# emdgroup/tnmf

Hardware: AMD Instinct MI355X
Metric: MU-iterations/sec (higher is better)
Workload: dtype f32

## Files before the change

### tnmf_amd/csrc/fft.h

```cpp
#pragma once
#include "common.h"

struct FftArgs {
    const void *src0, *src1, *src2;
    void *dst0, *dst1;
    long ps_src, ps_dst;
    int planes, rows, cols;
    int ld_src, ld_dst;
    int KX, KXP;
    int yoff, xoff;
    int N, M, C, Hy;
    int n0, ngroups, nper;
    int mgroups, mper;
    int clamp0;
    double reg;
};

enum FftOp {
    kFftRowsFwd = 0,
    kFftRowsInv,
    kFftRowsInv2,
    kFftRowsMu,
    kFftColsFwd,
    kFftColsInv,
    kFftContractR,
    kFftGradH,
    kFftGradW,
};

typedef int (*fft_run_fn)(int op, int dtype, const FftArgs *a, hipStream_t s);
#define TNMF_FFT_DECL(L) int fft_run_##L(int op, int dtype, const FftArgs *a, hipStream_t s)
TNMF_FFT_DECL(32);
TNMF_FFT_DECL(48);
TNMF_FFT_DECL(64);
TNMF_FFT_DECL(96);
TNMF_FFT_DECL(144);
TNMF_FFT_DECL(192);
TNMF_FFT_DECL(270);
TNMF_FFT_DECL(288);
TNMF_FFT_DECL(384);
TNMF_FFT_DECL(540);
TNMF_FFT_DECL(576);
#undef TNMF_FFT_DECL

bool mixed_has_reconstruct(const Geo &g, int dtype);
bool mixed_has_grad_W(const Geo &g, int dtype);
int mixed_reconstruct(const Geo &g, const void *Tsp, const void *WT, void *OT, int KX, int KXP, hipStream_t s);
int mixed_grad_W(const Geo &g, const void *Tsp, const void *VT, const void *RT, void *Gn, void *Gp, int KX, int KXP,
                 int ngroups, int nper, hipStream_t s);

int spectral_contract_R(const Geo &g, int dtype, const void *SH, const void *SW, void *SR, int Ly, int KX, int KXP,
                        hipStream_t s);
int spectral_grad_W(const Geo &g, int dtype, const void *SH, const void *SV, const void *SR, void *Gn, void *Gp, int Ly,
                    int KX, int KXP, int ngroups, int nper, hipStream_t s);

bool fft_has(const Geo &g, int dtype);
void fft_invalidate(tnmf_hip_ctx *ctx);
void fft_invalidate_H(tnmf_hip_ctx *ctx, const Geo &g, int dtype, const void *H);
void fft_bind(tnmf_hip_ctx *ctx, const Geo &g, int dtype, const void *H, const void *V);
void fft_unbind(tnmf_hip_ctx *ctx);
void fft_invalidate_W(tnmf_hip_ctx *ctx);
void fft_release(tnmf_hip_ctx *ctx);
int fft_reserve(tnmf_hip_ctx *ctx, const Geo &g, int dtype, bool with_window);

int fft_reconstruct(tnmf_hip_ctx *ctx, const Geo &g, int dtype, const void *W, const void *H, void *R, bool nonneg,
                    hipStream_t s);
int fft_grad_H(tnmf_hip_ctx *ctx, const Geo &g, int dtype, const void *V, const void *R, const void *W, void *neg,
               void *pos, hipStream_t s);
int fft_update_H(tnmf_hip_ctx *ctx, const Geo &g, int dtype, const void *V, const void *R, const void *W, void *H,
                 double reg, hipStream_t s);
int fft_grad_W(tnmf_hip_ctx *ctx, const Geo &g, int dtype, const void *V, const void *R, const void *H, void *neg,
               void *pos, bool nonneg, hipStream_t s);
```

### tnmf_amd/csrc/fft.hip

```cpp
#include <algorithm>
#include <cstdlib>

#include "fft.h"
#include "fft_engine.h"

namespace {

const int kLensY[] = {32, 48, 64, 96, 144, 192, 270, 288, 384, 576};
const int kLensX[] = {32, 48, 64, 96, 144, 192, 270, 288, 384, 540, 576};
constexpr int kMixMaxGroups = 128;

int pick_len(int h, int dtype, bool along_x, bool tall = false) {
    if (along_x || tall) {
        for (int L : kLensX)
            if (L >= h && (dtype == 0 || L <= 288)) return L;
        return 0;
    }
    for (int L : kLensY)
        if (L >= h && (dtype == 0 || L <= 288)) return L;
    return 0;
}

bool tall_columns(const tnmf_hip_ctx *ctx) { return ctx->path != TNMF_PATH_FFT; }

// ... 372 lines not shown
    a.planes = planes;
    a.rows = rows;
    a.cols = cols;
    a.ld_src = cols;
    a.ps_src = (long)rows * cols;
    a.ps_dst = (long)rows * l.KXP;
    return l.rowf(kFftRowsFwd, dtype, &a, s);
}

int columns_of(const Geo &g, const Lay &l, int dtype, const void *Tsrc, int planes, int rows, void *S, hipStream_t s) {
    FftArgs b = base_args(g, l);
    b.src0 = Tsrc;
    b.dst0 = S;
    b.planes = planes;
    b.rows = rows;
    return l.colf(kFftColsFwd, dtype, &b, s);
}

int spectra_V(tnmf_hip_ctx *ctx, const Geo &g, const Call &c, int dtype, const void *V, bool full, hipStream_t s) {
    FftState &f = ctx->fft;
    const Lay &l = c.l;
    const bool track = c.sl.v_cached && f.cache_enabled;
    const bool hit = track && all_ok(f.V_ok, c.sl.n0, g.N);
    ++(hit ? f.v_hits : f.v_runs);
    if (!track && c.sl.cached) {
        set_ok(f.V_ok, c.sl.n0, g.N, 0);
        set_ok(f.SV_ok, c.sl.n0, g.N, 0);
    }
    if (!hit) {
        if (track) {
            set_ok(f.V_ok, c.sl.n0, g.N, 0);
            set_ok(f.SV_ok, c.sl.n0, g.N, 0);
        }
        CHECK(forward_rows(g, l, dtype, V, g.N * g.C, g.Dy, g.Dx, c.VT, s));
        if (track) set_ok(f.V_ok, c.sl.n0, g.N, 1);
    }
    if (full && !(hit && all_ok(f.SV_ok, c.sl.n0, g.N))) {
        CHECK(columns_of(g, l, dtype, c.VT, g.N * g.C, g.Dy, c.SV, s));
        if (track) set_ok(f.SV_ok, c.sl.n0, g.N, 1);
    }
    return TNMF_OK;
}

int rows_of_H(tnmf_hip_ctx *ctx, const Geo &g, const Call &c, int dtype, const void *H, hipStream_t s) {
    FftState &f = ctx->fft;
    const bool track = c.sl.cached && f.cache_enabled;
    if (track && all_ok(f.T_ok, c.sl.n0, g.N)) {
        ++f.h_hits;
        return TNMF_OK;
    }
    ++f.h_runs;
    if (track) {
        set_ok(f.T_ok, c.sl.n0, g.N, 0);
        set_ok(f.SH_ok, c.sl.n0, g.N, 0);
    }
    FftArgs a = base_args(g, c.l);
    a.src0 = H;
    a.dst0 = c.T;
    a.planes = g.N * g.M;
    a.rows = g.Hy;
    a.cols = g.Hx;
    a.ld_src = g.Hs;
    a.ps_src = (long)g.Hy * g.Hs;
    a.ps_dst = (long)g.Hy * c.l.KXP;
    CHECK(c.l.rowf(kFftRowsFwd, dtype, &a, s));
    if (track) set_ok(f.T_ok, c.sl.n0, g.N, 1);
    return TNMF_OK;
}

int spectra_of_H(tnmf_hip_ctx *ctx, const Geo &g, const Call &c, int dtype, const void *H, hipStream_t s) {
    FftState &f = ctx->fft;
    CHECK(rows_of_H(ctx, g, c, dtype, H, s));
    const bool track = c.sl.cached && f.cache_enabled;
    if (track && all_ok(f.SH_ok, c.sl.n0, g.N)) return TNMF_OK;
    CHECK(columns_of(g, c.l, dtype, c.T, g.N * g.M, g.Hy, c.SH, s));
    if (track) set_ok(f.SH_ok, c.sl.n0, g.N, 1);
    return TNMF_OK;
}

}

bool fft_has(const Geo &g, int dtype) {
    if (g.Dy == 1 && g.Ay == 1) {
        return pick_len(g.Hx, dtype, true) != 0 && mixed_has_reconstruct(g, dtype) && mixed_has_grad_W(g, dtype);
    }
    return pick_len(g.Hy, dtype, false) != 0 && pick_len(g.Hx, dtype, true) != 0;
}

void fft_bind(tnmf_hip_ctx *ctx, const Geo &g, int dtype, const void *H, const void *V) {
    bind(ctx->fft, g, dtype, H, V, true);
}

void fft_unbind(tnmf_hip_ctx *ctx) {
    FftState &f = ctx->fft;
    f.bound = f.explicit_bind = false;
    f.H_base = f.V_base = nullptr;
    f.T_ok.clear();
    f.SH_ok.clear();
    f.V_ok.clear();
    f.SV_ok.clear();
}

void fft_invalidate_H(tnmf_hip_ctx *ctx, const Geo &g, int dtype, const void *H) {
    FftState &f = ctx->fft;
    const Slot sl = locate(f, g, dtype, H, nullptr);
    if (sl.cached) {
        set_ok(f.T_ok, sl.n0, g.N, 0);
        set_ok(f.SH_ok, sl.n0, g.N, 0);
    } else {
        std::fill(f.T_ok.begin(), f.T_ok.end(), 0);
        std::fill(f.SH_ok.begin(), f.SH_ok.end(), 0);
    }
}

void fft_invalidate(tnmf_hip_ctx *ctx) { clear_flags(ctx->fft); }

void fft_invalidate_W(tnmf_hip_ctx *ctx) { ctx->fft.W_ok = false; }

int fft_reserve(tnmf_hip_ctx *ctx, const Geo &g, int dtype, bool with_window) {
    Lay l;
    ctx->fft.failed_bytes = 0;
    const FftState &f = ctx->fft;
    const bool in_binding = f.bound && f.dtype == dtype && same_shape(f.geo, g) && f.geo.N >= g.N;
    if (!fft_has(g, dtype) || !make_layout(ctx, in_binding ? f.geo : g, g, dtype, &l)) return TNMF_E_UNSUPPORTED;
    return ensure_ws(ctx, with_window ? l.total : l.total_no_window);
}

void fft_release(tnmf_hip_ctx *ctx) {
    if (ctx->fft.ws) (void)hipFree(ctx->fft.ws);
    ctx->fft.ws = nullptr;
    ctx->fft.ws_bytes = 0;
    ctx->fft.failed_bytes = 0;
    clear_flags(ctx->fft);
}

int fft_reconstruct(tnmf_hip_ctx *ctx, const Geo &g, int dtype, const void *W, const void *H, void *R, bool nonneg,
                    hipStream_t s) {
    Call c;
    CHECK(prepare(ctx, g, dtype, H, nullptr, &c));
    const Lay &l = c.l;
    CHECK(rows_of_H(ctx, g, c, dtype, H, s));
    FftState &f = ctx->fft;
    const bool w_hit = f.cache_enabled && f.W_ok && f.W_owner == W && f.W_dtype == dtype && same_shape(f.W_geo, g) &&
                       (c.sl.cached || f.W_geo.N == g.N);
    auto w_mark = [&]() {
        f.W_ok = f.cache_enabled;
        f.W_owner = W;
        f.W_geo = g;
        f.W_dtype = dtype;
    };
    if (use_mixed(g, dtype, false)) {
        if (!w_hit) {
            f.W_ok = false;
            CHECK(scaled_W(ctx, g, l, dtype, W, 1.0 / l.Lx, s));
            CHECK(forward_rows(g, l, dtype, at(ctx, l.Wt), g.M * g.C, g.Ay, g.Ax, at(ctx, l.TWr), s));
            w_mark();
        }
        CHECK(mixed_reconstruct(g, c.T, at(ctx, l.TWr), c.Ts, l.KX, l.KXP, s));
    } else {
        if (!w_hit) {
            f.W_ok = false;
            CHECK(spectra_W(ctx, g, l, dtype, W, true, false, s));
            w_mark();
        }
        if (use_resident(l)) {
            CHECK(spectra_of_H(ctx, g, c, dtype, H, s));
            CHECK(spectral_contract_R(g, dtype, c.SH, at(ctx, l.SW), c.SR, l.Ly, l.KX, l.KXP, s));
        } else {
            FftArgs a = base_args(g, l);
            a.src0 = c.T;
            a.src1 = at(ctx, l.SW);
            a.dst0 = c.SR;
            CHECK(l.colf(kFftContractR, dtype, &a, s));
        }
        FftArgs b = base_args(g, l);
        b.src0 = c.SR;
        b.dst0 = c.Ts;
        b.planes = g.N * g.C;
        b.rows = g.Dy;
        b.yoff = g.Ay - 1;
        CHECK(l.colf(kFftColsInv, dtype, &b, s));
    }
    FftArgs d = base_args(g, l);
    d.src0 = c.Ts;
    d.dst0 = R;
    d.planes = g.N * g.C;
    d.rows = g.Dy;
    d.cols = g.Dx;
    d.xoff = g.Ax - 1;
    d.ld_dst = g.Dx;
    d.ps_dst = (long)g.Dy * g.Dx;
    d.clamp0 = nonneg ? 1 : 0;
    return l.rowf(kFftRowsInv, dtype, &d, s);
}

namespace {

int grad_H_spectra(tnmf_hip_ctx *ctx, const Geo &g, const Call &c, int dtype, const void *V, const void *R,
                   const void *W, hipStream_t s) {
    CHECK(spectra_W(ctx, g, c.l, dtype, W, false, true, s));
    CHECK(spectra_V(ctx, g, c, dtype, V, true, s));
    return forward_planes(g, c.l, dtype, R, g.N * g.C, g.Dy, g.Dx, c.Ts, c.SR, s);
}

int grad_H_window(tnmf_hip_ctx *ctx, const Geo &g, const Call &c, int dtype, int n0, int cnt, hipStream_t s) {
    const Lay &l = c.l;
    FftArgs a = base_args(g, l);
    a.src0 = c.SV;
    a.src1 = c.SR;
    a.src2 = at(ctx, l.SWf);
    a.dst0 = at(ctx, l.Tn);
    a.dst1 = at(ctx, l.Tp);
    a.n0 = n0;
    a.planes = cnt;
    a.mgroups = l.mgroups;
    a.mper = l.mper;
    return l.colf(kFftGradH, dtype, &a, s);
}

}

int fft_grad_H(tnmf_hip_ctx *ctx, const Geo &g, int dtype, const void *V, const void *R, const void *W, void *neg,
               void *pos, hipStream_t s) {
    if (g.Dy == 1 && g.Ay == 1) return TNMF_E_UNSUPPORTED;
    Call c;
    CHECK(prepare(ctx, g, dtype, nullptr, V, &c, true));
    const Lay &l = c.l;
    CHECK(grad_H_spectra(ctx, g, c, dtype, V, R, W, s));
    const size_t esz = l.csz / 2, hplane = (size_t)g.M * g.Hy * g.Hx;
    for (int n0 = 0; n0 < g.N; n0 += l.chunk) {
        const int cnt = g.N - n0 < l.chunk ? g.N - n0 : l.chunk;
        CHECK(grad_H_window(ctx, g, c, dtype, n0, cnt, s));
        FftArgs a = base_args(g, l);
        a.src0 = at(ctx, l.Tn);
        a.src1 = at(ctx, l.Tp);
        a.dst0 = static_cast<char *>(neg) + (size_t)n0 * hplane * esz;
        a.dst1 = static_cast<char *>(pos) + (size_t)n0 * hplane * esz;
        a.planes = cnt * g.M;
        a.rows = g.Hy;
        a.cols = g.Hx;
        a.xoff = 0;
        a.ld_dst = g.Hx;
        a.ps_dst = (long)g.Hy * g.Hx;
        CHECK(l.rowf(kFftRowsInv2, dtype, &a, s));
    }
    return TNMF_OK;
}

int fft_update_H(tnmf_hip_ctx *ctx, const Geo &g, int dtype, const void *V, const void *R, const void *W, void *H,
                 double reg, hipStream_t s) {
    if (g.Dy == 1 && g.Ay == 1) return TNMF_E_UNSUPPORTED;
    Call c;
    CHECK(prepare(ctx, g, dtype, H, V, &c, true));
    const Lay &l = c.l;
    FftState &f = ctx->fft;
    const bool track = c.sl.cached && f.cache_enabled;
    CHECK(grad_H_spectra(ctx, g, c, dtype, V, R, W, s));
    if (track) {
        set_ok(f.T_ok, c.sl.n0, g.N, 0);
        set_ok(f.SH_ok, c.sl.n0, g.N, 0);
    }
    const size_t esz = l.csz / 2, hplane = (size_t)g.M * g.Hy * g.Hs;
    for (int n0 = 0; n0 < g.N; n0 += l.chunk) {
        const int cnt = g.N - n0 < l.chunk ? g.N - n0 : l.chunk;
        CHECK(grad_H_window(ctx, g, c, dtype, n0, cnt, s));
        FftArgs a = base_args(g, l);
        a.src0 = at(ctx, l.Tn);
        a.src1 = at(ctx, l.Tp);
        a.dst0 = static_cast<char *>(H) + (size_t)n0 * hplane * esz;
        a.dst1 = c.T + (size_t)n0 * l.sT;
        a.planes = cnt * g.M;
        a.rows = g.Hy;
        a.cols = g.Hx;
        a.ld_dst = g.Hs;
        a.ps_src = (long)g.Hy * g.Hs;
        a.ps_dst = (long)g.Hy * l.KXP;
        a.reg = reg;
        CHECK(l.rowf(kFftRowsMu, dtype, &a, s));
    }
    if (track) set_ok(f.T_ok, c.sl.n0, g.N, 1);
    return TNMF_OK;
}

int mix_groups(const tnmf_hip_ctx *ctx, const Geo &g, const Lay &l) {
    const long slots = 2L * 4 * (ctx->num_cu > 0 ? ctx->num_cu : 256);
    const long per_group_block = (long)(g.C == 1 && g.Ay <= 12 ? cdiv(g.M, 2) : g.M) * cdiv(l.KX, 16);
    int best = 32;
    double best_cost = 1e30;
    for (int cand = 32; cand <= kMixMaxGroups; cand *= 2) {
        int ng = g.N < cand ? g.N : cand;
        const int nper = cdiv(g.N, ng);
        ng = cdiv(g.N, nper);
        const double rounds = (double)(per_group_block * cdiv(ng, 4)) / (double)slots;
        const double whole = rounds <= 1.0 ? 1.0 : (double)(long)(rounds + 0.999999);
        const double cost = whole / rounds + 0.03 * (cand / 32);
        if (cost < best_cost - 1e-9) {
            best_cost = cost;
            best = cand;
        }
    }
    return best;
}

int fft_grad_W(tnmf_hip_ctx *ctx, const Geo &g, int dtype, const void *V, const void *R, const void *H, void *neg,
               void *pos, bool nonneg, hipStream_t s) {
    Call c;
    CHECK(prepare(ctx, g, dtype, H, V, &c));
    const Lay &l = c.l;
    CHECK(rows_of_H(ctx, g, c, dtype, H, s));
    const bool mixed = use_mixed(g, dtype, true);
    CHECK(spectra_V(ctx, g, c, dtype, V, !mixed, s));
    const int planes = 2 * g.M * g.C;
    if (mixed) {
        CHECK(forward_rows(g, l, dtype, R, g.N * g.C, g.Dy, g.Dx, c.RT, s));
        int ng_want = mix_groups(ctx, g, l);
        if (const char *e = tnmf_diag_env("TNMF_MIX_GROUPS")) ng_want = atoi(e);
        ng_want = ng_want < 1 ? 1 : (ng_want > kMixMaxGroups ? kMixMaxGroups : ng_want);
        int ng = g.N < ng_want ? g.N : ng_want;
        const int nper = cdiv(g.N, ng);
        ng = cdiv(g.N, nper);
        const int ngpad = (int)align_up((size_t)ng, 4);
        CHECK(mixed_grad_W(g, c.T, c.VT, c.RT, at(ctx, l.Gn), at(ctx, l.Gp), l.KX, l.KXP, ngpad, nper, s));
        const long count = (long)g.M * g.C * g.Ay * l.KXP;
        char *out = at(ctx, l.TW);
        hipLaunchKernelGGL(k_fft_sum_groups<float>, dim3((unsigned)((count + 63) / 64), 2), dim3(64), 0, s,
                           (const cplx<float> *)at(ctx, l.Gn), (const cplx<float> *)at(ctx, l.Gp), (cplx<float> *)out,
                           (cplx<float> *)(out + (size_t)count * l.csz), count, ngpad, 1.0 / l.Lx);
        TNMF_LAUNCH_CHECK();
    } else {
        CHECK(forward_planes(g, l, dtype, R, g.N * g.C, g.Dy, g.Dx, c.Ts, c.SR, s));
        int ngroups = l.ngroups;
        if (use_resident(l)) {
            CHECK(spectra_of_H(ctx, g, c, dtype, H, s));
            const long blocks = (long)cdiv(g.M, 4) * (((long)l.Ly * l.KXP + 255) / 256) * cdiv(g.C, 4);
            int ng = (int)((8L * ctx->num_cu + blocks - 1) / blocks);
            ng = ng < 1 ? 1 : (ng > l.ngroups ? l.ngroups : ng);
            const int nper = cdiv(g.N, ng);
            ngroups = cdiv(g.N, nper);
            CHECK(spectral_grad_W(g, dtype, c.SH, c.SV, c.SR, at(ctx, l.Gn), at(ctx, l.Gp), l.Ly, l.KX, l.KXP, ngroups,
                                  nper, s));
        } else {
            FftArgs a = base_args(g, l);
            a.src0 = c.T;
            a.src1 = c.SV;
            a.src2 = c.SR;
            a.dst0 = at(ctx, l.Gn);
            a.dst1 = at(ctx, l.Gp);
            a.ngroups = l.ngroups;
            a.nper = l.nper;
            CHECK(l.colf(kFftGradW, dtype, &a, s));
        }
        const long count = (long)g.M * g.C * l.Ly * l.KXP;
        const size_t sbytes = (size_t)count * l.csz;
        const double scale = 1.0 / ((double)l.Ly * l.Lx);
        {
            char *out = at(ctx, l.Gs);
            const dim3 grid((unsigned)((count + 63) / 64), 2);
            if (dtype == 0)
                hipLaunchKernelGGL(k_fft_sum_groups<float>, grid, dim3(64), 0, s, (const cplx<float> *)at(ctx, l.Gn),
                                   (const cplx<float> *)at(ctx, l.Gp), (cplx<float> *)out, (cplx<float> *)(out + sbytes),
                                   count, ngroups, scale);
            else
                hipLaunchKernelGGL(k_fft_sum_groups<double>, grid, dim3(64), 0, s, (const cplx<double> *)at(ctx, l.Gn),
                                   (const cplx<double> *)at(ctx, l.Gp), (cplx<double> *)out,
                                   (cplx<double> *)(out + sbytes), count, ngroups, scale);
            TNMF_LAUNCH_CHECK();
        }
        FftArgs b = base_args(g, l);
        b.src0 = at(ctx, l.Gs);
        b.dst0 = at(ctx, l.TW);
        b.planes = planes;
        b.rows = g.Ay;
        b.yoff = 0;
        CHECK(l.colf(kFftColsInv, dtype, &b, s));
    }
    FftArgs d = base_args(g, l);
    d.src0 = at(ctx, l.TW);
    d.dst0 = at(ctx, l.Wo);
    d.planes = planes;
    d.rows = g.Ay;
    d.cols = g.Ax;
    d.xoff = 0;
    d.ld_dst = g.Ax;
    d.ps_dst = (long)g.Ay * g.Ax;
    CHECK(l.rowf(kFftRowsInv, dtype, &d, s));
    const int per = g.M * g.C * g.Ay * g.Ax;
    const char *wo = at(ctx, l.Wo);
    if (dtype == 0) {
        hipLaunchKernelGGL(k_fft_flip_out<float>, dim3(cdiv(per, 256)), dim3(256), 0, s, (const float *)wo,
                           (float *)neg, g.M * g.C, g.Ay, g.Ax, nonneg ? 1 : 0);
        hipLaunchKernelGGL(k_fft_flip_out<float>, dim3(cdiv(per, 256)), dim3(256), 0, s, (const float *)wo + per,
                           (float *)pos, g.M * g.C, g.Ay, g.Ax, nonneg ? 1 : 0);
    } else {
        hipLaunchKernelGGL(k_fft_flip_out<double>, dim3(cdiv(per, 256)), dim3(256), 0, s, (const double *)wo,
                           (double *)neg, g.M * g.C, g.Ay, g.Ax, nonneg ? 1 : 0);
        hipLaunchKernelGGL(k_fft_flip_out<double>, dim3(cdiv(per, 256)), dim3(256), 0, s, (const double *)wo + per,
                           (double *)pos, g.M * g.C, g.Ay, g.Ax, nonneg ? 1 : 0);
    }
    TNMF_LAUNCH_CHECK();
    return TNMF_OK;
}
```

### tnmf_amd/csrc/fft_mixed.hip

```cpp
#include "fft.h"

namespace {

typedef float f2v __attribute__((ext_vector_type(2)));
template <typename T>
struct cplx_of;
template <>
struct cplx_of<float> {
    using type = f2v;
};
template <typename T>
using cplx = typename cplx_of<T>::type;

__device__ __forceinline__ void cfma(f2v &acc, f2v a, f2v b) {
    asm("v_pk_fma_f32 %0, %1, %2, %0 op_sel:[0,0,0] op_sel_hi:[0,1,1]" : "+v"(acc) : "v"(a), "v"(b));
    asm("v_pk_fma_f32 %0, %1, %2, %0 op_sel:[1,1,0] op_sel_hi:[1,0,1] neg_lo:[0,1,0]" : "+v"(acc) : "v"(a), "v"(b));
}
__device__ __forceinline__ void cfmac(f2v &acc, f2v a, f2v b) {
    asm("v_pk_fma_f32 %0, %1, %2, %0 op_sel:[0,0,0] op_sel_hi:[0,1,1] neg_hi:[0,1,0]" : "+v"(acc) : "v"(a), "v"(b));
    asm("v_pk_fma_f32 %0, %1, %2, %0 op_sel:[1,1,0] op_sel_hi:[1,0,1]" : "+v"(acc) : "v"(a), "v"(b));
}

#define CHECK(rc_expr)                  \
    do {                                \
        const int _rc = (rc_expr);      \
        if (_rc != TNMF_OK) return _rc; \
    } while (0)

constexpr int kMixCols = 16;

template <typename T, int AY, int CG, int S, int STRIPS>
__global__ __launch_bounds__(kMixCols *STRIPS, 2) void k_mix_reconstruct(const cplx<T> *Tsp, const cplx<T> *WT,
                                                                      cplx<T> *OT, int M, int C, int Hy, int Dy, int KX,
                                                                      int KXP) {
    const int col = threadIdx.x & (kMixCols - 1), strip = threadIdx.x / kMixCols;
    const int kx = blockIdx.x * kMixCols + col, kxc = min(kx, KX - 1);
    const int y0 = (blockIdx.y * STRIPS + strip) * S, n = blockIdx.z;
    cplx<T> acc[CG][S];
#pragma unroll
    for (int c = 0; c < CG; ++c)
#pragma unroll
        for (int y = 0; y < S; ++y) acc[c][y] = {0, 0};
    static_assert(sizeof(cplx<T>) == 8, "float spectra");
    typedef unsigned u32x2v __attribute__((ext_vector_type(2)));
    auto ld = [](const __amdgpu_buffer_rsrc_t &rs, int lane_off, int row_off) {
        const u32x2v w2 = __builtin_amdgcn_raw_buffer_load_b64(rs, lane_off, row_off, 0);
        const unsigned re = w2[0], im = w2[1];
        return cplx<T>{__builtin_bit_cast(float, re), __builtin_bit_cast(float, im)};
    };
    const int rowb = KXP * 8;
    const long tplane = (long)Hy * KXP, wplane = (long)AY * KXP;
    const int lane_t = (y0 * KXP + kxc) * 8, lane_w = kxc * 8;
    const __amdgpu_buffer_rsrc_t wrs =
        __builtin_amdgcn_make_buffer_rsrc((void *)WT, 0, (int)((long)M * C * wplane * 8), 0x00020000);
    auto plane = [&](int m) {
        return __builtin_amdgcn_make_buffer_rsrc((void *)(Tsp + ((long)n * M + m) * tplane), 0, (int)(tplane * 8),
                                                 0x00020000);
    };
    cplx<T> t[S + AY - 1], tn[S + AY - 1];
    {
        const __amdgpu_buffer_rsrc_t rs = plane(0);
#pragma unroll
        for (int r = 0; r < S + AY - 1; ++r) t[r] = ld(rs, lane_t, r * rowb);
    }
    if constexpr (CG == 1) {
        constexpr int MC = 8, NT = kMixCols * STRIPS, ROWS = MC * AY, PIECES = ROWS * (kMixCols / 2);
        constexpr int NPP = (PIECES + NT - 1) / NT;
        typedef float f4v __attribute__((ext_vector_type(4)));
        __shared__ __align__(16) cplx<T> wl[2][ROWS * kMixCols];
        const cplx<T> *wsrc = WT + blockIdx.x * kMixCols;
        const int wrows = M * AY;
        f4v pre[NPP];
        auto wfetch = [&](int chunk) {
#pragma unroll
            for (int k = 0; k < NPP; ++k) {
                const int p = threadIdx.x + k * NT, row = min(chunk * ROWS + (p >> 3), wrows - 1);
                pre[k] = *reinterpret_cast<const f4v *>(wsrc + (long)row * KXP + 2 * (p & 7));
            }
        };
        auto wpark = [&](int buf) {
#pragma unroll
            for (int k = 0; k < NPP; ++k) {
                const int p = threadIdx.x + k * NT;
                if (p < PIECES) *reinterpret_cast<f4v *>(&wl[buf][(p >> 3) * kMixCols + 2 * (p & 7)]) = pre[k];
            }
        };
        wfetch(0);
        wpark(0);
        __syncthreads();
#pragma unroll 1
        for (int m0 = 0, ch = 0; m0 < M; m0 += MC, ++ch) {
            const int buf = ch & 1;
            const bool more = m0 + MC < M;
            if (more) wfetch(ch + 1);
#pragma unroll 1
            for (int mi = 0; mi < MC; ++mi) {
                const int m = m0 + mi;
                if (m >= M) break;
                cplx<T> w[AY];
#pragma unroll
                for (int a = 0; a < AY; ++a) w[a] = wl[buf][(mi * AY + (AY - 1 - a)) * kMixCols + col];
                {
                    const __amdgpu_buffer_rsrc_t rs = plane(min(m + 1, M - 1));
#pragma unroll
                    for (int r = 0; r < S + AY - 1; ++r) tn[r] = ld(rs, lane_t, r * rowb);
                }
#pragma unroll
                for (int a = 0; a < AY; ++a)
#pragma unroll
                    for (int y = 0; y < S; ++y) cfma(acc[0][y], t[y + a], w[a]);
#pragma unroll
                for (int r = 0; r < S + AY - 1; ++r) t[r] = tn[r];
            }
            if (more) wpark(buf ^ 1);
            __syncthreads();
        }
    } else {
#pragma unroll 1
    for (int m = 0; m < M; ++m) {
        cplx<T> w[CG][AY];
#pragma unroll
        for (int c = 0; c < CG; ++c) {
            const int wbase = ((m * C + min(c, C - 1)) * AY) * rowb;
#pragma unroll
            for (int a = 0; a < AY; ++a) w[c][a] = ld(wrs, lane_w, wbase + (AY - 1 - a) * rowb);
        }
        {
            const __amdgpu_buffer_rsrc_t rs = plane(min(m + 1, M - 1));
#pragma unroll
            for (int r = 0; r < S + AY - 1; ++r) tn[r] = ld(rs, lane_t, r * rowb);
        }
#pragma unroll
        for (int c = 0; c < CG; ++c)
#pragma unroll
            for (int a = 0; a < AY; ++a)
#pragma unroll
                for (int y = 0; y < S; ++y) cfma(acc[c][y], t[y + a], w[c][a]);
#pragma unroll
        for (int r = 0; r < S + AY - 1; ++r) t[r] = tn[r];
    }
    }
    if (kx >= KX) return;
#pragma unroll
    for (int c = 0; c < CG; ++c) {
        if (c >= C) break;
#pragma unroll
        for (int y = 0; y < S; ++y)
            if (y0 + y < Dy) OT[((long)n * C + c) * ((long)Dy * KXP) + (long)(y0 + y) * KXP + kx] = acc[c][y];
    }
}

template <typename T, int CG, int SAMPLES>
__global__ __launch_bounds__(kMixCols *SAMPLES) void k_mix_reconstruct_1d(const cplx<T> *Tsp, const cplx<T> *WT,
                                                                        cplx<T> *OT, int N, int M, int C, int KX,
                                                                        int KXP) {
    const int col = threadIdx.x & (kMixCols - 1), sub = threadIdx.x / kMixCols;
    const int kx = blockIdx.x * kMixCols + col, kxc = min(kx, KX - 1);
    const int n = blockIdx.y * SAMPLES + sub, nc = min(n, N - 1);
    cplx<T> acc[CG];
#pragma unroll
    for (int c = 0; c < CG; ++c) acc[c] = {0, 0};
    const cplx<T> *tp = Tsp + (long)nc * M * KXP + kxc;
    int m = 0;
    for (; m + 4 <= M; m += 4) {
        cplx<T> t[4];
#pragma unroll
        for (int q = 0; q < 4; ++q) t[q] = tp[(long)(m + q) * KXP];
#pragma unroll
        for (int q = 0; q < 4; ++q)
#pragma unroll
            for (int c = 0; c < CG; ++c) cfma(acc[c], t[q], WT[((long)(m + q) * C + min(c, C - 1)) * KXP + kxc]);
    }
    for (; m < M; ++m) {
        const cplx<T> t = tp[(long)m * KXP];
#pragma unroll
        for (int c = 0; c < CG; ++c) cfma(acc[c], t, WT[((long)m * C + min(c, C - 1)) * KXP + kxc]);
    }
    if (kx >= KX || n >= N) return;
#pragma unroll
    for (int c = 0; c < CG; ++c) {
        if (c >= C) break;
        OT[((long)n * C + c) * KXP + kx] = acc[c];
    }
}

template <typename T, int AY>
int launch_mix_reconstruct(const void *Tsp, const void *WT, void *OT, const Geo &g, int KX, int KXP, hipStream_t s) {
    const unsigned tiles = (unsigned)cdiv(KX, kMixCols);
    if constexpr (AY == 1) {
        if (g.Dy == 1) {
            constexpr int SAMPLES = 16;
            hipLaunchKernelGGL((k_mix_reconstruct_1d<T, 3, SAMPLES>), dim3(tiles, (unsigned)cdiv(g.N, SAMPLES)),
                               dim3(kMixCols * SAMPLES), 0, s, (const cplx<T> *)Tsp, (const cplx<T> *)WT, (cplx<T> *)OT,
                               g.N, g.M, g.C, KX, KXP);
            TNMF_LAUNCH_CHECK();
            return TNMF_OK;
        }
    }
    if (g.C == 1) {
        constexpr int S = 16, STRIPS = 8;
        hipLaunchKernelGGL((k_mix_reconstruct<T, AY, 1, S, STRIPS>),
                           dim3(tiles, (unsigned)cdiv(g.Dy, S * STRIPS), (unsigned)g.N), dim3(kMixCols * STRIPS), 0, s,
                           (const cplx<T> *)Tsp, (const cplx<T> *)WT, (cplx<T> *)OT, g.M, g.C, g.Hy, g.Dy, KX, KXP);
    } else {
        constexpr int S = 8, STRIPS = 8;
        hipLaunchKernelGGL((k_mix_reconstruct<T, AY, 3, S, STRIPS>),
                           dim3(tiles, (unsigned)cdiv(g.Dy, S * STRIPS), (unsigned)g.N), dim3(kMixCols * STRIPS), 0, s,
                           (const cplx<T> *)Tsp, (const cplx<T> *)WT, (cplx<T> *)OT, g.M, g.C, g.Hy, g.Dy, KX, KXP);
    }
    TNMF_LAUNCH_CHECK();
    return TNMF_OK;
}

template <typename T, int AY, int CG, int GROUPS>
__global__ __launch_bounds__(kMixCols *GROUPS, 2) void k_mix_grad_W(const cplx<T> *Tsp, const cplx<T> *VT,
                                                                 const cplx<T> *RT, cplx<T> *Gn, cplx<T> *Gp, int N,
                                                                 int M, int C, int Hy, int Dy, int KX, int KXP,
                                                                 int nper) {
    const int col = threadIdx.x & (kMixCols - 1), sub = threadIdx.x / kMixCols;
    const int kx = blockIdx.y * kMixCols + col, kxc = min(kx, KX - 1);
    const int m = blockIdx.x, grp = blockIdx.z * GROUPS + sub;
    cplx<T> an[CG][AY], ap[CG][AY];
#pragma unroll
    for (int c = 0; c < CG; ++c)
#pragma unroll
        for (int a = 0; a < AY; ++a) {
            an[c][a] = {0, 0};
            ap[c][a] = {0, 0};
        }
    const int nbeg = grp * nper, nend = min(N, nbeg + nper);
    const long tplane = (long)Hy * KXP, vplane = (long)Dy * KXP;
    static_assert(CG == 1, "one channel per thread");
#pragma unroll 1
    for (int n = nbeg; n < nend; ++n) {
        const cplx<T> *tp = Tsp + ((long)n * M + m) * tplane;
        const cplx<T> *vp = VT + (long)n * C * vplane, *rp = RT + (long)n * C * vplane;
        cplx<T> t[2 * AY - 1], v[AY], r[AY], tn[AY], vn[AY], rn[AY];
#pragma unroll
        for (int i = 0; i < 2 * AY - 1; ++i) t[i] = tp[(unsigned)(min(i, Hy - 1) * KXP + kxc)];
#pragma unroll
        for (int j = 0; j < AY; ++j) {
            const unsigned o = (unsigned)(min(j, Dy - 1) * KXP + kxc);
            v[j] = vp[o];
            r[j] = rp[o];
        }
#pragma unroll 1
        for (int yb = 0; yb < Dy; yb += AY) {
#pragma unroll
            for (int i = 0; i < AY; ++i) tn[i] = tp[(unsigned)(min(yb + 2 * AY - 1 + i, Hy - 1) * KXP + kxc)];
#pragma unroll
            for (int j = 0; j < AY; ++j) {
                const unsigned o = (unsigned)(min(yb + AY + j, Dy - 1) * KXP + kxc);
                vn[j] = vp[o];
                rn[j] = rp[o];
            }
#pragma unroll
            for (int j = 0; j < AY; ++j) {
                if (yb + j >= Dy) {
                    v[j] = {0, 0};
                    r[j] = {0, 0};
                }
#pragma unroll
                for (int a = 0; a < AY; ++a) {
                    cfmac(an[0][a], t[j + a], v[j]);
                    cfmac(ap[0][a], t[j + a], r[j]);
                }
            }
#pragma unroll
            for (int i = 0; i < AY - 1; ++i) t[i] = t[i + AY];
#pragma unroll
            for (int i = 0; i < AY; ++i) t[AY - 1 + i] = tn[i];
#pragma unroll
            for (int j = 0; j < AY; ++j) {
                v[j] = vn[j];
                r[j] = rn[j];
            }
        }
    }
    if (kx >= KX) return;
    const long gplane = (long)AY * KXP, gsize = (long)M * C * gplane;
#pragma unroll
    for (int c = 0; c < CG; ++c) {
        if (c >= C) break;
#pragma unroll
        for (int a = 0; a < AY; ++a) {
            const long o = (long)grp * gsize + ((long)m * C + c) * gplane + (long)a * KXP + kx;
            Gn[o] = an[c][a];
            Gp[o] = ap[c][a];
        }
    }
}

template <typename T, int AY, int GROUPS>
__global__ __launch_bounds__(kMixCols *GROUPS, 2) void k_mix_grad_W2(const cplx<T> *Tsp, const cplx<T> *VT,
                                                                  const cplx<T> *RT, cplx<T> *Gn, cplx<T> *Gp, int N,
                                                                  int M, int Hy, int Dy, int KX, int KXP, int nper,
                                                                  int gx, int gy, int gz) {
    constexpr int MA = 2, VS = 8, RS = (AY + 4 + VS - 1) / VS * VS, P = VS - 1;
    const int col = threadIdx.x & (kMixCols - 1), sub = threadIdx.x / kMixCols;
    int lin = blockIdx.x;
    {
        const int total = gx * gy * gz, whole = total / 8 * 8;
        if (lin < whole) lin = (lin & 7) * (whole / 8) + (lin >> 3);
    }
    const int bx = lin % gx, by = (lin / gx) % gy, bz = lin / (gx * gy);
    const int kx = by * kMixCols + col, kxc = min(kx, KX - 1);
    const int m0 = bx * MA, grp = bz * GROUPS + sub;
    const int m1 = min(m0 + 1, M - 1);
    cplx<T> an[MA][AY], ap[MA][AY];
#pragma unroll
    for (int q = 0; q < MA; ++q)
#pragma unroll
        for (int a = 0; a < AY; ++a) {
            an[q][a] = {0, 0};
            ap[q][a] = {0, 0};
        }
    static_assert(sizeof(cplx<T>) == 8, "float spectra");
    typedef unsigned u32x2v __attribute__((ext_vector_type(2)));
    const long tplane = (long)Hy * KXP, vplane = (long)Dy * KXP;
    const int nbeg0 = bz * GROUPS * nper, nbeg = nbeg0 + sub * nper;
    const int lane_t = (int)(((long)sub * nper * M * tplane + kxc) * 8);
    const int lane_v = (int)(((long)sub * nper * vplane + kxc) * 8);
    const int rowb = KXP * 8;
    auto ld = [](const __amdgpu_buffer_rsrc_t &rs, int lane_off, int row_off) {
        const u32x2v w = __builtin_amdgcn_raw_buffer_load_b64(rs, lane_off, row_off, 0);
        const unsigned re = w[0], im = w[1];
        return cplx<T>{__builtin_bit_cast(float, re), __builtin_bit_cast(float, im)};
    };
#pragma unroll 1
    for (int nr = 0; nr < nper; ++nr) {
        if (nbeg0 + nr >= N) break;
        if (nbeg + nr >= N) continue;
        const cplx<T> *tb = Tsp + ((long)(nbeg0 + nr) * M + m0) * tplane;
        const __amdgpu_buffer_rsrc_t t0 = __builtin_amdgcn_make_buffer_rsrc((void *)tb, 0, 0x7fffffff, 0x00020000);
        const __amdgpu_buffer_rsrc_t t1 =
            __builtin_amdgcn_make_buffer_rsrc((void *)(tb + (long)(m1 - m0) * tplane), 0, 0x7fffffff, 0x00020000);
        const __amdgpu_buffer_rsrc_t vb =
            __builtin_amdgcn_make_buffer_rsrc((void *)(VT + (long)(nbeg0 + nr) * vplane), 0, 0x7fffffff, 0x00020000);
        const __amdgpu_buffer_rsrc_t rb =
            __builtin_amdgcn_make_buffer_rsrc((void *)(RT + (long)(nbeg0 + nr) * vplane), 0, 0x7fffffff, 0x00020000);
        cplx<T> t[MA][RS], v[VS], r[VS];
#pragma unroll
        for (int i = 0; i < RS - 1; ++i) {
            const int o = min(i, Hy - 1) * rowb;
            t[0][i] = ld(t0, lane_t, o);
            t[1][i] = ld(t1, lane_t, o);
        }
#pragma unroll
        for (int i = 0; i < P; ++i) {
            const int o = min(i, Dy - 1) * rowb;
            v[i] = ld(vb, lane_v, o);
            r[i] = ld(rb, lane_v, o);
        }
#pragma unroll 1
        for (int yb = 0; yb < Dy; yb += RS) {
#pragma unroll
            for (int i = 0; i < RS; ++i) {
                const int y = yb + i;
                if (y >= Dy) break;
                {
                    const int o = min(y + RS - 1, Hy - 1) * rowb;
                    t[0][(i + RS - 1) % RS] = ld(t0, lane_t, o);
                    t[1][(i + RS - 1) % RS] = ld(t1, lane_t, o);
                    const int ov = min(y + P, Dy - 1) * rowb;
                    v[(i + P) % VS] = ld(vb, lane_v, ov);
                    r[(i + P) % VS] = ld(rb, lane_v, ov);
                }
                const cplx<T> vy = v[i % VS], ry = r[i % VS];
#pragma unroll
                for (int a = 0; a < AY; ++a) {
                    cfmac(an[0][a], t[0][(i + a) % RS], vy);
                    cfmac(ap[0][a], t[0][(i + a) % RS], ry);
                    cfmac(an[1][a], t[1][(i + a) % RS], vy);
                    cfmac(ap[1][a], t[1][(i + a) % RS], ry);
                }
            }
        }
    }
    if (kx >= KX) return;
    const long gplane = (long)AY * KXP, gsize = (long)M * gplane;
#pragma unroll
    for (int q = 0; q < MA; ++q) {
        if (m0 + q >= M) break;
#pragma unroll
        for (int a = 0; a < AY; ++a) {
            const long o = (long)grp * gsize + (long)(m0 + q) * gplane + (long)a * KXP + kx;
            Gn[o] = an[q][a];
            Gp[o] = ap[q][a];
        }
    }
}

template <typename T, int CG, int GROUPS>
__global__ __launch_bounds__(kMixCols *GROUPS) void k_mix_grad_W_1d(const cplx<T> *Tsp, const cplx<T> *VT, const cplx<T> *RT,
                                                                  cplx<T> *Gn, cplx<T> *Gp, int N, int M, int C, int KX,
                                                                  int KXP, int nper) {
    const int col = threadIdx.x & (kMixCols - 1), sub = threadIdx.x / kMixCols;
    const int kx = blockIdx.y * kMixCols + col, kxc = min(kx, KX - 1);
    const int m = blockIdx.x, grp = blockIdx.z * GROUPS + sub;
    cplx<T> an[CG], ap[CG];
#pragma unroll
    for (int c = 0; c < CG; ++c) {
        an[c] = {0, 0};
        ap[c] = {0, 0};
    }
    const int nbeg = grp * nper, nend = min(N, nbeg + nper);
    for (int n = nbeg; n < nend; ++n) {
        const cplx<T> t = Tsp[((long)n * M + m) * KXP + kxc];
#pragma unroll
        for (int c = 0; c < CG; ++c) {
            const long o = ((long)n * C + min(c, C - 1)) * KXP + kxc;
            cfmac(an[c], t, VT[o]);
            cfmac(ap[c], t, RT[o]);
        }
    }
    if (kx >= KX) return;
    const long gsize = (long)M * C * KXP;
#pragma unroll
    for (int c = 0; c < CG; ++c) {
        if (c >= C) break;
        const long o = (long)grp * gsize + ((long)m * C + c) * KXP + kx;
        Gn[o] = an[c];
        Gp[o] = ap[c];
    }
}

template <typename T, int AY>
int launch_mix_grad_W(const void *Tsp, const void *VT, const void *RT, void *Gn, void *Gp, const Geo &g, int KX,
                      int KXP, int ngroups, int nper, hipStream_t s) {
    constexpr int GROUPS = 4;
    if constexpr (AY == 1) {
        if (g.Dy == 1) {
            const dim3 grid((unsigned)g.M, (unsigned)cdiv(KX, kMixCols), (unsigned)cdiv(ngroups, GROUPS));
            hipLaunchKernelGGL((k_mix_grad_W_1d<T, 4, GROUPS>), grid, dim3(kMixCols * GROUPS), 0, s, (const cplx<T> *)Tsp,
                               (const cplx<T> *)VT, (const cplx<T> *)RT, (cplx<T> *)Gn, (cplx<T> *)Gp, g.N, g.M, g.C, KX,
                               KXP, nper);
            TNMF_LAUNCH_CHECK();
            return TNMF_OK;
        }
    }
    if constexpr (AY <= 12) {
        const long span = ((long)(GROUPS - 1) * nper * g.M + 2) * g.Hy * KXP * 8;
        if (g.C == 1 && span < (1L << 31)) {
            const int gx = cdiv(g.M, 2), gy = cdiv(KX, kMixCols), gz = cdiv(ngroups, GROUPS);
            hipLaunchKernelGGL((k_mix_grad_W2<T, AY, GROUPS>), dim3((unsigned)(gx * gy * gz)), dim3(kMixCols * GROUPS), 0, s,
                               (const cplx<T> *)Tsp, (const cplx<T> *)VT, (const cplx<T> *)RT, (cplx<T> *)Gn,
                               (cplx<T> *)Gp, g.N, g.M, g.Hy, g.Dy, KX, KXP, nper, gx, gy, gz);
            TNMF_LAUNCH_CHECK();
            return TNMF_OK;
        }
    }
    const dim3 grid((unsigned)g.M, (unsigned)cdiv(KX, kMixCols), (unsigned)cdiv(ngroups, GROUPS));
    hipLaunchKernelGGL((k_mix_grad_W<T, AY, 1, GROUPS>), grid, dim3(kMixCols * GROUPS), 0, s, (const cplx<T> *)Tsp,
                       (const cplx<T> *)VT, (const cplx<T> *)RT, (cplx<T> *)Gn, (cplx<T> *)Gp, g.N, g.M, g.C, g.Hy, g.Dy,
                       KX, KXP, nper);
    TNMF_LAUNCH_CHECK();
    return TNMF_OK;
}

#define MIX_SWITCH(FN, ...)                                   \
    switch (g.Ay) {                                           \
        case 1: return FN<float, 1>(__VA_ARGS__);             \
        case 2: return FN<float, 2>(__VA_ARGS__);             \
        case 3: return FN<float, 3>(__VA_ARGS__);             \
        case 4: return FN<float, 4>(__VA_ARGS__);             \
        case 5: return FN<float, 5>(__VA_ARGS__);             \
        case 6: return FN<float, 6>(__VA_ARGS__);             \
        case 7: return FN<float, 7>(__VA_ARGS__);             \
        case 8: return FN<float, 8>(__VA_ARGS__);             \
        case 9: return FN<float, 9>(__VA_ARGS__);             \
        case 10: return FN<float, 10>(__VA_ARGS__);           \
        case 11: return FN<float, 11>(__VA_ARGS__);           \
        case 12: return FN<float, 12>(__VA_ARGS__);           \
        case 13: return FN<float, 13>(__VA_ARGS__);           \
        case 14: return FN<float, 14>(__VA_ARGS__);           \
        case 15: return FN<float, 15>(__VA_ARGS__);           \
        case 16: return FN<float, 16>(__VA_ARGS__);           \
        default: return TNMF_E_UNSUPPORTED;                   \
    }

}

bool mixed_has_reconstruct(const Geo &g, int dtype) {
    return dtype == 0 && g.Ay <= 16 && (g.C == 1 || (g.Dy == 1 && g.Ay == 1 && g.C <= 3));
}
bool mixed_has_grad_W(const Geo &g, int dtype) {
    return dtype == 0 && g.Ay <= 16 && (g.C == 1 || (g.Dy == 1 && g.Ay == 1 && g.C <= 4));
}

int mixed_reconstruct(const Geo &g, const void *Tsp, const void *WT, void *OT, int KX, int KXP, hipStream_t s) {
    MIX_SWITCH(launch_mix_reconstruct, Tsp, WT, OT, g, KX, KXP, s);
}

int mixed_grad_W(const Geo &g, const void *Tsp, const void *VT, const void *RT, void *Gn, void *Gp, int KX, int KXP,
                 int ngroups, int nper, hipStream_t s) {
    MIX_SWITCH(launch_mix_grad_W, Tsp, VT, RT, Gn, Gp, g, KX, KXP, ngroups, nper, s);
}
```

Before: 208.6.

## Add LDS-staged grad_W kernel with 16 atoms per block and Karatsuba-style products

Adds a new mixed grad_W kernel that handles 16 atoms per block. V and R rows are staged in double-buffered shared memory, and each thread keeps a register ring of T rows loaded through buffer-resource loads. The complex products are computed in a three-multiply form (c, c+d, c−d) using packed FMAs, and the group count is chosen by a new occupancy cost model. The aim is more reuse of V/R across atoms and less arithmetic for large spectra. In exchange the kernel is complex, uses more registers and LDS, and only runs when C=1, Ay≤12 and the spectra are large.

Result: faster. 214.7 (median of 6 runs) (+2.9%).

```diff
diff --git a/tnmf_amd/csrc/fft.h b/tnmf_amd/csrc/fft.h
--- a/tnmf_amd/csrc/fft.h
+++ b/tnmf_amd/csrc/fft.h
@@ -49,6 +49,17 @@
 int mixed_grad_W(const Geo &g, const void *Tsp, const void *VT, const void *RT, void *Gn, void *Gp, int KX, int KXP,
                  int ngroups, int nper, hipStream_t s);
 
+#ifndef TNMF_MIX_W3_WAVES
+#define TNMF_MIX_W3_WAVES 3
+#endif
+constexpr int kMixW3Atoms = 16, kMixW3Waves = TNMF_MIX_W3_WAVES, kMixW3MaxAy = 12;
+constexpr long kMixW3MinBytes = 24L << 20;
+constexpr int mix_w3_waves(int Ay) {
+    const int w = Ay >= 8 ? 3 : (Ay >= 4 ? 4 : (Ay >= 2 ? 5 : 7));
+    return kMixW3Waves < 3 ? kMixW3Waves : w;
+}
+bool mixed_grad_W3_takes(const Geo &g, int KXP);
+
 int spectral_contract_R(const Geo &g, int dtype, const void *SH, const void *SW, void *SR, int Ly, int KX, int KXP,
                         hipStream_t s);
 int spectral_grad_W(const Geo &g, int dtype, const void *SH, const void *SV, const void *SR, void *Gn, void *Gp, int Ly,
diff --git a/tnmf_amd/csrc/fft.hip b/tnmf_amd/csrc/fft.hip
--- a/tnmf_amd/csrc/fft.hip
+++ b/tnmf_amd/csrc/fft.hip
@@ -698,6 +698,24 @@
     return best;
 }
 
+int mix_groups_w3(const tnmf_hip_ctx *ctx, const Geo &g, const Lay &l) {
+    const long slots3 = (long)mix_w3_waves(g.Ay) * (ctx->num_cu > 0 ? ctx->num_cu : 256);
+    const long per_group = (long)cdiv(g.M, kMixW3Atoms) * cdiv(l.KX, 16);
+    int best = 1;
+    double best_cost = 1e30;
+    for (int cand = g.N < kMixMaxGroups ? g.N : kMixMaxGroups; cand >= 1; --cand) {
+        const int ng = cdiv(g.N, cdiv(g.N, cand));
+        const double rounds = (double)(per_group * ng) / (double)slots3;
+        const double whole = rounds <= 1.0 ? 1.0 : (double)(long)(rounds + 0.999999);
+        const double cost3 = whole / rounds + 0.03 * ng / 32.0;
+        if (cost3 < best_cost - 1e-9) {
+            best_cost = cost3;
+            best = ng;
+        }
+    }
+    return best;
+}
+
 int fft_grad_W(tnmf_hip_ctx *ctx, const Geo &g, int dtype, const void *V, const void *R, const void *H, void *neg,
                void *pos, bool nonneg, hipStream_t s) {
     Call c;
@@ -716,12 +734,17 @@
         const int nper = cdiv(g.N, ng);
         ng = cdiv(g.N, nper);
         const int ngpad = (int)align_up((size_t)ng, 4);
-        CHECK(mixed_grad_W(g, c.T, c.VT, c.RT, at(ctx, l.Gn), at(ctx, l.Gp), l.KX, l.KXP, ngpad, nper, s));
+        int nparts = ngpad, nper_call = nper;
+        if (mixed_grad_W3_takes(g, l.KXP)) {
+            nper_call = cdiv(g.N, mix_groups_w3(ctx, g, l));
+            nparts = cdiv(g.N, nper_call);
+        }
+        CHECK(mixed_grad_W(g, c.T, c.VT, c.RT, at(ctx, l.Gn), at(ctx, l.Gp), l.KX, l.KXP, nparts, nper_call, s));
         const long count = (long)g.M * g.C * g.Ay * l.KXP;
         char *out = at(ctx, l.TW);
         hipLaunchKernelGGL(k_fft_sum_groups<float>, dim3((unsigned)((count + 63) / 64), 2), dim3(64), 0, s,
                            (const cplx<float> *)at(ctx, l.Gn), (const cplx<float> *)at(ctx, l.Gp), (cplx<float> *)out,
-                           (cplx<float> *)(out + (size_t)count * l.csz), count, ngpad, 1.0 / l.Lx);
+                           (cplx<float> *)(out + (size_t)count * l.csz), count, nparts, 1.0 / l.Lx);
         TNMF_LAUNCH_CHECK();
     } else {
         CHECK(forward_planes(g, l, dtype, R, g.N * g.C, g.Dy, g.Dx, c.Ts, c.SR, s));
diff --git a/tnmf_amd/csrc/fft_mixed.hip b/tnmf_amd/csrc/fft_mixed.hip
--- a/tnmf_amd/csrc/fft_mixed.hip
+++ b/tnmf_amd/csrc/fft_mixed.hip
@@ -19,6 +19,12 @@
 __device__ __forceinline__ void cfmac(f2v &acc, f2v a, f2v b) {
     asm("v_pk_fma_f32 %0, %1, %2, %0 op_sel:[0,0,0] op_sel_hi:[0,1,1] neg_hi:[0,1,0]" : "+v"(acc) : "v"(a), "v"(b));
     asm("v_pk_fma_f32 %0, %1, %2, %0 op_sel:[1,1,0] op_sel_hi:[1,0,1]" : "+v"(acc) : "v"(a), "v"(b));
+}
+__device__ __forceinline__ void pfma_lo(f2v &acc, f2v x, f2v b) {
+    asm("v_pk_fma_f32 %0, %1, %2, %0 op_sel:[0,0,0] op_sel_hi:[1,0,1]" : "+v"(acc) : "v"(x), "v"(b));
+}
+__device__ __forceinline__ void pfma_hi(f2v &acc, f2v x, f2v b) {
+    asm("v_pk_fma_f32 %0, %1, %2, %0 op_sel:[0,1,0] op_sel_hi:[1,1,1]" : "+v"(acc) : "v"(x), "v"(b));
 }
 
 #define CHECK(rc_expr)                  \
@@ -391,6 +397,117 @@
     }
 }
 
+#if defined(__HIP_DEVICE_COMPILE__)
+#define TNMF_MIX_NO_DS_PAIRING __attribute__((target("no-load-store-opt")))
+#else
+#define TNMF_MIX_NO_DS_PAIRING
+#endif
+template <typename T, int AY>
+__global__ __launch_bounds__(kMixCols *kMixW3Atoms, kMixW3Waves) TNMF_MIX_NO_DS_PAIRING void k_mix_grad_W3(
+    const cplx<T> *Tsp, const cplx<T> *VT, const cplx<T> *RT, cplx<T> *Gn, cplx<T> *Gp, int N, int M, int Hy, int Dy,
+    int KX, int KXP, int nper, int gx, int gy, int gz) {
+    constexpr int NA = kMixW3Atoms, RS = 16, CH = RS, NT = kMixCols * NA;
+    static_assert(AY + 4 <= RS && sizeof(cplx<T>) == 8 && NT == 2 * CH * (kMixCols / 2), "ring depth, float spectra");
+    const int col = threadIdx.x & (kMixCols - 1), slot = threadIdx.x / kMixCols;
+    int lin = blockIdx.x;
+    {
+        const int total = gx * gy * gz, whole = total / 8 * 8;
+        if (lin < whole) lin = (lin & 7) * (whole / 8) + (lin >> 3);
+    }
+    const int bx = lin % gx, by = (lin / gx) % gy, grp = lin / (gx * gy);
+    const int kx = by * kMixCols + col, kxc = min(kx, KX - 1);
+    const int m = bx * NA + slot, mc = min(m, M - 1);
+    f2v a1[AY], a2[AY], a3[AY];
+#pragma unroll
+    for (int a = 0; a < AY; ++a) a1[a] = a2[a] = a3[a] = {0, 0};
+    typedef unsigned u32x2v __attribute__((ext_vector_type(2)));
+    typedef float f4v __attribute__((ext_vector_type(4)));
+    const long tplane = (long)Hy * KXP, vplane = (long)Dy * KXP;
+    const int nbeg = grp * nper, nend = min(N, nbeg + nper);
+    const int lane_t = (int)(((long)(mc - bx * NA) * tplane + kxc) * 8);
+    const int rowb = KXP * 8;
+    auto ld = [](const __amdgpu_buffer_rsrc_t &rs, int lane_off, int row_off) {
+        const u32x2v w = __builtin_amdgcn_raw_buffer_load_b64(rs, lane_off, row_off, 0);
+        const unsigned re = w[0], im = w[1];
+        return cplx<T>{__builtin_bit_cast(float, re), __builtin_bit_cast(float, im)};
+    };
+    __shared__ __align__(16) f2v xl[2][3][CH * kMixCols];
+    const int prow = threadIdx.x / kMixCols, ppair = (threadIdx.x >> 1) & (kMixCols / 2 - 1), pstream = threadIdx.x & 1;
+    const cplx<T> *xsrc = (pstream ? RT : VT) + by * kMixCols + 2 * ppair;
+    f4v pre;
+    auto xfetch = [&](int n, int chunk) {
+        pre = *reinterpret_cast<const f4v *>(xsrc + (long)n * vplane + (long)min(chunk * CH + prow, Dy - 1) * KXP);
+    };
+    auto xpark = [&](int buf) {
+        auto swap1 = [](float v) {
+            return __builtin_bit_cast(float,
+                                      __builtin_amdgcn_update_dpp(0, __builtin_bit_cast(int, v), 0xB1, 0xf, 0xf, false));
+        };
+        const float oc = swap1(pstream ? pre[0] : pre[2]), od = swap1(pstream ? pre[1] : pre[3]);
+        const float cv = pstream ? oc : pre[0], dv = pstream ? od : pre[1];
+        const float cr = pstream ? pre[2] : oc, dr = pstream ? pre[3] : od;
+        const int e = prow * kMixCols + 2 * ppair + pstream;
+        xl[buf][0][e] = f2v{cv, cr};
+        xl[buf][1][e] = f2v{cv + dv, cr + dr};
+        xl[buf][2][e] = f2v{cv - dv, cr - dr};
+    };
+    xfetch(min(nbeg, N - 1), 0);
+    xpark(0);
+    __syncthreads();
+    int buf = 0;
+#pragma unroll 1
+    for (int n = nbeg; n < nend; ++n) {
+        const __amdgpu_buffer_rsrc_t t0 = __builtin_amdgcn_make_buffer_rsrc(
+            (void *)(Tsp + ((long)n * M + bx * NA) * tplane), 0, 0x7fffffff, 0x00020000);
+        cplx<T> t[RS];
+        f2v sp[RS / 2];
+#pragma unroll
+        for (int i = 0; i < RS - 1; ++i) t[i] = ld(t0, lane_t, min(i, Hy - 1) * rowb);
+#pragma unroll
+        for (int i = 0; i < AY - 1; ++i) sp[i / 2][i & 1] = t[i][0] + t[i][1];
+#pragma unroll 1
+        for (int yb = 0; yb < Dy; yb += CH) {
+            {
+                const bool last = yb + CH >= Dy;
+                xfetch(last ? min(n + 1, nend - 1) : n, last ? 0 : yb / CH + 1);
+            }
+            const f2v *x1 = &xl[buf][0][col], *x2 = &xl[buf][1][col], *x3 = &xl[buf][2][col];
+#pragma unroll
+            for (int i = 0; i < RS; ++i) {
+                const int y = yb + i;
+                if (y >= Dy) break;
+                t[(i + RS - 1) % RS] = ld(t0, lane_t, min(y + RS - 1, Hy - 1) * rowb);
+                {
+                    const int j = (i + AY - 1) % RS;
+                    sp[j / 2][j & 1] = t[j][0] + t[j][1];
+                }
+                const f2v c = x1[i * kMixCols], cpd = x2[i * kMixCols], cmd = x3[i * kMixCols];
+#pragma unroll
+                for (int a = 0; a < AY; ++a) {
+                    const int j = (i + a) % RS;
+                    if (j & 1)
+                        pfma_hi(a1[a], c, sp[j / 2]);
+                    else
+                        pfma_lo(a1[a], c, sp[j / 2]);
+                    pfma_lo(a2[a], cpd, t[j]);
+                    pfma_hi(a3[a], cmd, t[j]);
+                }
+            }
+            xpark(buf ^ 1);
+            __syncthreads();
+            buf ^= 1;
+        }
+    }
+    if (kx >= KX || m >= M) return;
+    const long gplane = (long)AY * KXP, gsize = (long)M * gplane;
+#pragma unroll
+    for (int a = 0; a < AY; ++a) {
+        const long o = (long)grp * gsize + (long)m * gplane + (long)a * KXP + kx;
+        Gn[o] = cplx<T>{a1[a][0] - a3[a][0], a1[a][0] - a2[a][0]};
+        Gp[o] = cplx<T>{a1[a][1] - a3[a][1], a1[a][1] - a2[a][1]};
+    }
+}
+
 template <typename T, int CG, int GROUPS>
 __global__ __launch_bounds__(kMixCols *GROUPS) void k_mix_grad_W_1d(const cplx<T> *Tsp, const cplx<T> *VT, const cplx<T> *RT,
                                                                   cplx<T> *Gn, cplx<T> *Gp, int N, int M, int C, int KX,
@@ -435,6 +552,17 @@
             hipLaunchKernelGGL((k_mix_grad_W_1d<T, 4, GROUPS>), grid, dim3(kMixCols * GROUPS), 0, s, (const cplx<T> *)Tsp,
                                (const cplx<T> *)VT, (const cplx<T> *)RT, (cplx<T> *)Gn, (cplx<T> *)Gp, g.N, g.M, g.C, KX,
                                KXP, nper);
+            TNMF_LAUNCH_CHECK();
+            return TNMF_OK;
+        }
+    }
+    if constexpr (AY <= kMixW3MaxAy) {
+        if (mixed_grad_W3_takes(g, KXP)) {
+            const int gx = cdiv(g.M, kMixW3Atoms), gy = cdiv(KX, kMixCols), gz = ngroups;
+            hipLaunchKernelGGL((k_mix_grad_W3<T, AY>), dim3((unsigned)(gx * gy * gz)), dim3(kMixCols * kMixW3Atoms),
+                               kMixW3Waves == 2 ? 48u << 10 : 0u, s,
+                               (const cplx<T> *)Tsp, (const cplx<T> *)VT, (const cplx<T> *)RT, (cplx<T> *)Gn,
+                               (cplx<T> *)Gp, g.N, g.M, g.Hy, g.Dy, KX, KXP, nper, gx, gy, gz);
             TNMF_LAUNCH_CHECK();
             return TNMF_OK;
         }
@@ -488,6 +616,15 @@
     return dtype == 0 && g.Ay <= 16 && (g.C == 1 || (g.Dy == 1 && g.Ay == 1 && g.C <= 4));
 }
 
+bool mixed_grad_W3_takes(const Geo &g, int KXP) {
+#ifdef TNMF_MIX_NO_W3
+    return false;
+#endif
+    const long span = (long)kMixW3Atoms * g.Hy * KXP * 8;
+    const long spectra = (long)g.N * g.M * g.Hy * KXP * 8;
+    return g.C == 1 && g.Ay <= kMixW3MaxAy && !(g.Dy == 1 && g.Ay == 1) && span < (1L << 31) && spectra >= kMixW3MinBytes;
+}
+
 int mixed_reconstruct(const Geo &g, const void *Tsp, const void *WT, void *OT, int KX, int KXP, hipStream_t s) {
     MIX_SWITCH(launch_mix_reconstruct, Tsp, WT, OT, g, KX, KXP, s);
 }
```
